# StevenChang5/Canny_Edge

Hardware: AMD Instinct MI355X
Metric: Mpixels/s device-resident Canny (4K gray, frames in HBM, whole pipeline); % HBM roofline on Sobel+NMS in `roofline`; the end-to-end (host->host, PCIe-inclusive) rate is `end_to_end` (higher is better)
Workload: dtype f32+s16; 1 GPU; 128x 3840x2160 gray frames per GPU per step, sigma=1.4, thresholds 50/150, inputs resident in HBM; frames_per_gpu=128, height=2160, width=3840

## Files before the change

### canny_edge_amd/csrc/canny_kernels.hip

```cpp
#include "canny_kernels.h"

#include <hip/hip_ext.h>

namespace canny {

__device__ __forceinline__ uint64_t shfl_up_u64(uint64_t v)
{
    unsigned lo = (unsigned)v, hi = (unsigned)(v >> 32);
    lo = __shfl_up(lo, 1);
    hi = __shfl_up(hi, 1);
    return ((uint64_t)hi << 32) | lo;
}
__device__ __forceinline__ uint64_t shfl_down_u64(uint64_t v)
{
    unsigned lo = (unsigned)v, hi = (unsigned)(v >> 32);
    lo = __shfl_down(lo, 1);
    hi = __shfl_down(hi, 1);
    return ((uint64_t)hi << 32) | lo;
}

__device__ __forceinline__ uint64_t readlane_u64(uint64_t v, int uniform_lane)
{
    const unsigned lo = (unsigned)__builtin_amdgcn_readlane((int)(unsigned)v, uniform_lane);
    const unsigned hi = (unsigned)__builtin_amdgcn_readlane((int)(unsigned)(v >> 32), uniform_lane);
    return ((uint64_t)hi << 32) | lo;
}

__device__ __forceinline__ uint64_t lane_u64(uint64_t v, int src_lane)
{
    unsigned lo = __shfl((unsigned)v, src_lane), hi = __shfl((unsigned)(v >> 32), src_lane);
    return ((uint64_t)hi << 32) | lo;
}

__device__ __forceinline__ int magnitude_general(int gx, int gy)
{
    long long n = (long long)gx * gx + (long long)gy * gy;
    return (int)(int16_t)(int)sqrt((double)n);
}
__device__ __forceinline__ int angle_bin_general(int gx, int gy)
{
    long long A = (long long)gx * gx, B = (long long)gy * gy, P = (long long)gx * gy;
    long long twoP = 2 * (P < 0 ? -P : P);
    if (twoP <= A - B) return 0;
    if (twoP < B - A) return 90;
    return P > 0 ? 45 : 135;
}
__device__ __forceinline__ int magnitude_d8(int gx, int gy)
{
    int n = __mul24(gx, gx) + __mul24(gy, gy);
    return (int)__builtin_amdgcn_sqrtf((float)n + 0.5f);
}
__device__ __forceinline__ int angle_bin_d8(int gx, int gy)
{
    int A = __mul24(gx, gx), B = __mul24(gy, gy), P = __mul24(gx, gy);
    int twoP = 2 * (P < 0 ? -P : P);
    int D = A - B;
    return (twoP <= D) ? 0 : ((twoP < -D) ? 90 : (P > 0 ? 45 : 135));
}

__device__ __forceinline__ void sobel_at(const int16_t *__restrict__ f, int H, int W, int r, int c, int &gx, int &gy)
{
    int cl = c > 0 ? c - 1 : 0, cr = c < W - 1 ? c + 1 : W - 1;
    int ru = r > 0 ? r - 1 : 0, rd = r < H - 1 ? r + 1 : H - 1;
    const int16_t *row = f + (size_t)r * W;
    const int16_t *up = f + (size_t)ru * W;
    const int16_t *dn = f + (size_t)rd * W;
    int v = 2 * row[cr] - 2 * row[cl];
    if (r < H - 1) v += dn[cr] - dn[cl];
    if (r > 0) v += up[cr] - up[cl];
    int u = 2 * dn[c] - 2 * up[c];
    if (c < W - 1) u += dn[c + 1] - up[c + 1];
    if (c > 0) u += dn[c - 1] - up[c - 1];
    gx = (int16_t)v;
    gy = (int16_t)u;
}

template <class At>
__device__ __forceinline__ void sobel_staged(const At &at, int H, int W, int r, int c, int ly, int lx, int &gx, int &gy)
{
    int lxl = c > 0 ? lx - 1 : lx, lxr = c < W - 1 ? lx + 1 : lx;
    int lyu = r > 0 ? ly - 1 : ly, lyd = r < H - 1 ? ly + 1 : ly;
    int v = 2 * at(ly, lxr) - 2 * at(ly, lxl);
    if (r < H - 1) v += at(ly + 1, lxr) - at(ly + 1, lxl);
    if (r > 0) v += at(ly - 1, lxr) - at(ly - 1, lxl);
    int u = 2 * at(lyd, lx) - 2 * at(lyu, lx);
    if (c < W - 1) u += at(lyd, lx + 1) - at(lyu, lx + 1);
    if (c > 0) u += at(lyd, lx - 1) - at(lyu, lx - 1);
    gx = (int16_t)v;
    gy = (int16_t)u;
}

__global__ __launch_bounds__(256) void gauss_rows_generic_kernel(const uint8_t *__restrict__ img,
                                                                 float *__restrict__ tmp, int W, size_t total,
                                                                 GaussTaps t)
{
    size_t stride = (size_t)gridDim.x * blockDim.x;
    for (size_t i = (size_t)blockIdx.x * blockDim.x + threadIdx.x; i < total; i += stride) {
        int c = (int)(i % (size_t)W);
        const uint8_t *row = img + (i - c);
        float acc = 0.0f, wsum = 0.0f;
        for (int k = -t.center; k <= t.center; k++) {
            int cc = c + k;
            if (cc >= 0 && cc < W) {
                float w = t.tap[t.center + k];
                acc = __fadd_rn(acc, __fmul_rn((float)row[cc], w));
                wsum = __fadd_rn(wsum, w);
            }
        }
        tmp[i] = __fdiv_rn(acc, wsum);
    }
}

__global__ __launch_bounds__(256) void gauss_cols_generic_kernel(const float *__restrict__ tmp,
                                                                 int16_t *__restrict__ out, int H, int W,
                                                                 size_t total, GaussTaps t)
{
    size_t stride = (size_t)gridDim.x * blockDim.x;
    for (size_t i = (size_t)blockIdx.x * blockDim.x + threadIdx.x; i < total; i += stride) {
        size_t rowidx = i / (size_t)W;
        int r = (int)(rowidx % (size_t)H);
        float acc = 0.0f, wsum = 0.0f;
        for (int k = -t.center; k <= t.center; k++) {
            int rr = r + k;
            if (rr >= 0 && rr < H) {
                float w = t.tap[t.center + k];
                acc = __fadd_rn(acc, __fmul_rn(tmp[i + (ptrdiff_t)k * W], w));
                wsum = __fadd_rn(wsum, w);
            }
        }
        out[i] = (int16_t)__fdiv_rn(acc, wsum);
    }
}

static inline unsigned grid_for(size_t total, int block, unsigned cap = 256u * 32u)
{
    size_t g = (total + block - 1) / block;
    if (g > cap) g = cap;
    if (g < 1) g = 1;
    return (unsigned)g;
}

hipError_t launch_gaussian_generic(const uint8_t *img, float *tmp, int16_t *out, int height, int width,
                                   int n_frames, const GaussTaps &taps, hipStream_t stream)
{
    size_t total = (size_t)n_frames * height * width;
    unsigned grid = grid_for(total, 256);
    hipLaunchKernelGGL(gauss_rows_generic_kernel, dim3(grid), dim3(256), 0, stream, img, tmp, width, total, taps);
    hipLaunchKernelGGL(gauss_cols_generic_kernel, dim3(grid), dim3(256), 0, stream, tmp, out, height, width, total,
                       taps);
    return hipGetLastError();
}


// ... 278 lines not shown
    int v[HG_PER_THREAD];
    auto fetch = [&](int t) {
        const int x0 = (t % tiles_x) * HG_TW, y0 = (t / tiles_x) * HG_TH;
#pragma unroll
        for (int k = 0; k < HG_PER_THREAD; k++) {
            const int i = (int)threadIdx.x + k * kHistWaves * 64;
            const int ly = i / (HG_TW + 2), lx = i - ly * (HG_TW + 2);
            const int r = y0 - 1 + ly, c = x0 - 1 + lx;
            v[k] = 0;
            if (t < tiles && i < HG_STAGE && r >= 0 && r < H && c >= 0 && c < W) {
                const size_t q = f * frame_px + (size_t)r * W + c;
                v[k] = U8 ? ((const uint8_t *)plane)[q] : ((const int16_t *)plane)[q];
            }
        }
    };
    fetch(blockIdx.x);
    for (int t = blockIdx.x; t < tiles; t += gridDim.x) {
        const int x0 = (t % tiles_x) * HG_TW, y0 = (t / tiles_x) * HG_TH;
        __syncthreads();
#pragma unroll
        for (int k = 0; k < HG_PER_THREAD; k++) {
            const int i = (int)threadIdx.x + k * kHistWaves * 64;
            if (i < HG_STAGE) (&tile[0][0])[i] = (int16_t)v[k];
        }
        __syncthreads();
        fetch(t + gridDim.x);
        for (int i = threadIdx.x; i < HG_TH * HG_TW; i += blockDim.x) {
            const int my = i / HG_TW, mx = i - my * HG_TW;
            const int r = y0 + my, c = x0 + mx;
            if (r >= H || c >= W) continue;
            int gx, gy;
            sobel_staged([&](int y, int x) -> int { return tile[y][x]; }, H, W, r, c, my + 1, mx + 1, gx, gy);
            wave_hist_add(h, min(magnitude_d8(gx, gy), kHistBins - 1));
        }
    }
    hist_flush(sh, hist + f * kHistBins);
}

static unsigned hist_blocks_per_frame(int n_frames, size_t units_per_frame)
{
    size_t b = ((size_t)kHistBlocks + n_frames - 1) / n_frames;
    if (b > units_per_frame) b = units_per_frame;
    return (unsigned)(b < 1 ? 1 : b);
}

hipError_t launch_hist_intensity(const void *plane, bool in_u8, uint32_t *hist, int height, int width, int n_frames,
                                 hipStream_t stream)
{
    const size_t frame_px = (size_t)height * width, total = frame_px * n_frames;
    const size_t lanes = (frame_px / 16 + 2 + kHistGroups - 1) / kHistGroups;
    const dim3 grid(hist_blocks_per_frame(n_frames, (lanes + kHistWaves * 64 - 1) / (kHistWaves * 64)), n_frames);
    if (in_u8)
        hipLaunchKernelGGL(hist_intensity_kernel<true>, grid, dim3(kHistWaves * 64), 0, stream, plane, hist, frame_px,
                           total);
    else
        hipLaunchKernelGGL(hist_intensity_kernel<false>, grid, dim3(kHistWaves * 64), 0, stream, plane, hist, frame_px,
                           total);
    return hipGetLastError();
}

hipError_t launch_hist_gradient(const void *plane, bool in_u8, uint32_t *hist, int height, int width, int n_frames,
                                hipStream_t stream)
{
    const size_t tiles = (size_t)((width + HG_TW - 1) / HG_TW) * ((height + HG_TH - 1) / HG_TH);
    const dim3 grid(hist_blocks_per_frame(n_frames, tiles), n_frames);
    if (in_u8)
        hipLaunchKernelGGL(hist_gradient_kernel<true>, grid, dim3(kHistWaves * 64), 0, stream, plane, hist, height,
                           width);
    else
        hipLaunchKernelGGL(hist_gradient_kernel<false>, grid, dim3(kHistWaves * 64), 0, stream, plane, hist, height,
                           width);
    return hipGetLastError();
}

__global__ __launch_bounds__(64) void thr_select_kernel(const uint32_t *__restrict__ hist, int rule, double low,
                                                        double high, int *__restrict__ pairs)
{
    __shared__ unsigned long long cs[kHistBins];
    const int f = blockIdx.x, lane = threadIdx.x;
    const uint32_t *hf = hist + (size_t)f * kHistBins;
    unsigned long long part[5], run = 0;
#pragma unroll
    for (int k = 0; k < 5; k++) {
        const int b = 5 * lane + k;
        run += b < kHistBins ? hf[b] : 0u;
        part[k] = run;
    }
    unsigned long long x = run;
    for (int d = 1; d < 64; d <<= 1) {
        const unsigned lo = __shfl_up((unsigned)x, d), hi = __shfl_up((unsigned)(x >> 32), d);
        if (lane >= d) x += ((unsigned long long)hi << 32) | lo;
    }
    const unsigned long long excl = x - run;
#pragma unroll
    for (int k = 0; k < 5; k++)
        if (5 * lane + k < kHistBins) cs[5 * lane + k] = excl + part[k];
    __syncthreads();
    if (lane == 0) {
        int lo, hi;
        auto_thresholds([&](int b) { return cs[b]; }, rule, low, high, lo, hi);
        pairs[2 * f] = lo;
        pairs[2 * f + 1] = hi;
    }
}

hipError_t launch_thr_select(const uint32_t *hist, int n_frames, int rule, double low, double high, int *pairs,
                             hipStream_t stream)
{
    hipLaunchKernelGGL(thr_select_kernel, dim3(n_frames), dim3(64), 0, stream, hist, rule, low, high, pairs);
    return hipGetLastError();
}

__device__ __forceinline__ size_t word_index(const HystGeom &g, int f, int y, int wx)
{
    return ((((size_t)f * g.tiles_y + (y >> 6)) * g.tiles_x + wx) << 6) + (y & 63);
}

template <bool THR>
__global__ __launch_bounds__(256) void hyst_classify_kernel(const int16_t *__restrict__ cand,
                                                            uint64_t *__restrict__ strong,
                                                            uint64_t *__restrict__ conn, HystGeom g, int lo, int hi,
                                                            unsigned *domain_flag, const int *__restrict__ pairs)
{
    const int lane = threadIdx.x & 63;
    const size_t rows_padded = (size_t)g.tiles_y * kTile;
    const size_t n_words = (size_t)g.n_frames * rows_padded * g.tiles_x;
    const size_t wave_stride = ((size_t)gridDim.x * blockDim.x) >> 6;
    for (size_t wv = ((size_t)blockIdx.x * blockDim.x + threadIdx.x) >> 6; wv < n_words; wv += wave_stride) {
        int wx = (int)(wv % (size_t)g.tiles_x);
        size_t t = wv / (size_t)g.tiles_x;
        int y = (int)(t % rows_padded);
        int f = (int)(t / rows_padded);
        if constexpr (THR) {
            lo = pairs[2 * f];
            hi = pairs[2 * f + 1];
            clamp_thresholds(lo, hi);
        }
        int x = wx * kTile + lane;
        bool inside = (y < g.height) && (x < g.width);
        int v = 0;
        if (inside) v = cand[((size_t)f * g.height + y) * g.width + x];
        bool c = inside && v >= lo;
        bool s = c && v >= hi;
        if (inside && lo <= 0 && v < lo) atomicOr(domain_flag, 1u);
        uint64_t mc = __ballot(c), ms = __ballot(s);
        if (lane == 0) {
            size_t idx = word_index(g, f, y, wx);
            conn[idx] = mc;
            strong[idx] = ms;
        }
    }
}

__device__ __forceinline__ uint64_t row_above_u64(uint64_t v)
{
    unsigned lo = (unsigned)__builtin_amdgcn_mov_dpp((int)(unsigned)v, 0x138 , 0xf, 0xf, true);
    unsigned hi = (unsigned)__builtin_amdgcn_mov_dpp((int)(unsigned)(v >> 32), 0x138, 0xf, 0xf, true);
    return ((uint64_t)hi << 32) | lo;
}
__device__ __forceinline__ uint64_t row_below_u64(uint64_t v)
{
    unsigned lo = (unsigned)__builtin_amdgcn_mov_dpp((int)(unsigned)v, 0x130 , 0xf, 0xf, true);
    unsigned hi = (unsigned)__builtin_amdgcn_mov_dpp((int)(unsigned)(v >> 32), 0x130, 0xf, 0xf, true);
    return ((uint64_t)hi << 32) | lo;
}

__device__ __forceinline__ uint64_t fill_runs(uint64_t p, uint64_t g)
{
    const uint64_t up = ((p + g) ^ p) & p;
    const uint64_t pr = __brevll(p), gr = __brevll(g);
    const uint64_t down = __brevll(((pr + gr) ^ pr) & pr);
    return g | up | down;
}

struct HystSched {
    unsigned *stamp, *queue0, *queue1, *count;
    unsigned *fq0, *fq1, *fcount;
};
constexpr int kSweep0Tiles = 2;
__device__ __forceinline__ HystSched make_sched(unsigned *words, int tiles)
{
    HystSched s;
    s.stamp = words;
    s.queue0 = words + tiles;
    s.queue1 = words + 2 * (size_t)tiles;
    s.count = words + 3 * (size_t)tiles;
    s.fq0 = words + 3 * (size_t)tiles + 4;
    s.fq1 = words + 4 * (size_t)tiles + 4;
    s.fcount = words + 5 * (size_t)tiles + 4;
    return s;
}

struct TileIn {
    uint64_t s0, su, sd;
    unsigned lb, rb;
    unsigned ul, ur, dl, dr;
};

constexpr uint64_t kAllHalo = ~0ull;
__device__ __forceinline__ TileIn load_tile(int t, int lane, const uint64_t *__restrict__ strong, const HystGeom &g,
                                            uint64_t c = kAllHalo)
{
    const int tpf = g.tiles_x * g.tiles_y;
    const int tt = t % tpf;
    const int ty = tt / g.tiles_x, tx = tt - ty * g.tiles_x;
    const uint64_t c_top = readlane_u64(c, 0), c_bot = readlane_u64(c, 63);
    const bool needL = __any((c & 1ull) != 0), needR = __any((c >> 63) != 0);
    const bool hasU = ty > 0 && c_top != 0, hasD = ty < g.tiles_y - 1 && c_bot != 0;
    const bool hasL = tx > 0 && needL, hasR = tx < g.tiles_x - 1 && needR;
    const size_t base = (size_t)t * kTile;
    const size_t rowstep = (size_t)g.tiles_x * kTile;
    TileIn in;
    in.s0 = strong[base + lane];
    in.su = hasU ? strong[base - rowstep + 63] : 0;
    in.sd = hasD ? strong[base + rowstep] : 0;
    in.lb = hasL ? (unsigned)(strong[base - kTile + lane] >> 63) : 0u;
    in.rb = hasR ? (unsigned)(strong[base + kTile + lane] & 1u) : 0u;
    in.ul = (hasU && hasL && (c_top & 1ull)) ? (unsigned)(strong[base - rowstep - kTile + 63] >> 63) : 0u;
    in.ur = (hasU && hasR && (c_top >> 63)) ? (unsigned)(strong[base - rowstep + kTile + 63] & 1u) : 0u;
    in.dl = (hasD && hasL && (c_bot & 1ull)) ? (unsigned)(strong[base + rowstep - kTile] >> 63) : 0u;
    in.dr = (hasD && hasR && (c_bot >> 63)) ? (unsigned)(strong[base + rowstep + kTile] & 1u) : 0u;
    return in;
}

__device__ __forceinline__ void push_neighbours(bool want, int lane, unsigned *stamp, unsigned slot, unsigned entry,
                                                unsigned nxt, unsigned *q, unsigned *cnt)
{
    const bool won = want && atomicExch(&stamp[slot], nxt) != nxt;
    const uint64_t winners = __ballot(won);
    if (winners == 0) return;
    unsigned first = 0;
    if (lane == 0) first = atomicAdd(cnt, (unsigned)__popcll(winners));
    first = (unsigned)__builtin_amdgcn_readlane((int)first, 0);
    if (won) q[first + (unsigned)__popcll(winners & ((1ull << lane) - 1ull))] = entry;
}

template <class Push>
__device__ __forceinline__ void process_tile_with(int t, int lane, uint64_t *__restrict__ strong, int iter,
                                                  const HystGeom &g, int16_t *__restrict__ edges, int edge_value,
                                                  uint64_t c, const TileIn &in, Push push_tiles)
{
    const int tpf = g.tiles_x * g.tiles_y;
    const int tt = t % tpf;
    const int ty = tt / g.tiles_x, tx = tt - ty * g.tiles_x;
    const bool hasU = ty > 0, hasD = ty < g.tiles_y - 1, hasL = tx > 0, hasR = tx < g.tiles_x - 1;
    const size_t base = (size_t)t * kTile;
    const uint64_t s0 = in.s0, su = in.su, sd = in.sd;
    const unsigned lb = in.lb, rb = in.rb, ul = in.ul, ur = in.ur, dl = in.dl, dr = in.dr;
    unsigned lb_up = __shfl_up(lb, 1), lb_dn = __shfl_down(lb, 1);
    unsigned rb_up = __shfl_up(rb, 1), rb_dn = __shfl_down(rb, 1);
    if (lane == 0) { lb_up = ul; rb_up = ur; }
    if (lane == 63) { lb_dn = dl; rb_dn = dr; }
    const uint64_t in_left = (uint64_t)(lb | lb_up | lb_dn);
    const uint64_t in_right = (uint64_t)(rb | rb_up | rb_dn) << 63;
    const bool quirk = (ty == 0 && tx == 0 && lane == 0);

    uint64_t s = s0;
    for (;;) {
        uint64_t up = row_above_u64(s), dn = row_below_u64(s);
        if (lane == 0) up = su;
        if (lane == 63) dn = sd;
        uint64_t d = up | s | dn;
        uint64_t d_from_left = quirk ? (up | s | (dn & ~1ull)) : d;
        uint64_t nb = d | (d_from_left << 1) | (d >> 1) | in_left | in_right;
        uint64_t gsel = s | (c & nb);
        if (!__any(gsel != s)) break;
        s = fill_runs(c, gsel);
    }

    const uint64_t chg = s ^ s0;
    const uint64_t rows_changed = __ballot(chg != 0);
    if (rows_changed != 0) {
        strong[base + lane] = s;
        if (edges) {
            const int f = t / tpf;
            const int cols = min(kTile, g.width - tx * kTile), rows = min(kTile, g.height - ty * kTile);
            int16_t *const tile0 = edges + ((size_t)f * g.height + (size_t)ty * kTile) * g.width + tx * kTile;
            if (__popcll(rows_changed) <= 16) {
                for (uint64_t m = rows_changed; m != 0; m &= m - 1) {
                    const int r = __builtin_ctzll(m);
                    const uint64_t word = readlane_u64(chg, r);
                    if (((word >> lane) & 1ull) != 0 && lane < cols && r < rows)
                        tile0[(size_t)r * g.width + lane] = (int16_t)edge_value;
                }
            } else if (lane < rows) {
                int16_t *const rowp = tile0 + (size_t)lane * g.width;
                for (uint64_t m = chg; m != 0; m &= m - 1) {
                    const int b = __builtin_ctzll(m);
                    if (b < cols) rowp[b] = (int16_t)edge_value;
                }
            }
        }
        const uint64_t top64 = readlane_u64(chg, 0);
        const uint64_t bot = readlane_u64(chg, 63);
        const bool anyL = __any((chg & 1ull) != 0), anyR = __any((chg >> 63) != 0);
        const int dy = (lane == 0 || lane == 4 || lane == 5) ? -1 : ((lane == 1 || lane == 6 || lane == 7) ? 1 : 0);
        const int dx = (lane == 2 || lane == 4 || lane == 6) ? -1 : ((lane == 3 || lane == 5 || lane == 7) ? 1 : 0);
        const uint64_t facing = dy < 0 ? top64 : bot;
        const bool hit = dy == 0 ? (dx < 0 ? anyL : anyR)
                                 : (dx == 0 ? facing != 0 : (dx < 0 ? (facing & 1ull) != 0 : (facing >> 63) != 0));
        const bool there = (dy >= 0 || hasU) && (dy <= 0 || hasD) && (dx >= 0 || hasL) && (dx <= 0 || hasR);
        const bool want = lane < 8 && hit && there;
        push_tiles(want, t + dy * g.tiles_x + dx);
    }
}

__device__ __forceinline__ void note_push(unsigned *last_change, unsigned nxt)
{
    if (__hip_atomic_load(last_change, __ATOMIC_RELAXED, __HIP_MEMORY_SCOPE_AGENT) < nxt) atomicMax(last_change, nxt);
}

__device__ __forceinline__ void process_tile(int t, int lane, uint64_t *__restrict__ strong, const HystSched &sch,
                                             unsigned *__restrict__ last_change, int iter, const HystGeom &g,
                                             int16_t *__restrict__ edges, int edge_value, uint64_t c,
                                             const TileIn &in, bool to_frame = false)
{
    const unsigned nxt = (unsigned)iter + 1u;
    unsigned *q = (nxt & 1u) ? sch.queue1 : sch.queue0;
    unsigned *cnt = sch.count + nxt % 3u;
    if (to_frame) {
        const int tpf = g.tiles_x * g.tiles_y;
        const int f = t / tpf;
        q = ((nxt & 1u) ? sch.fq1 : sch.fq0) + (size_t)f * tpf;
        cnt = sch.fcount + 4 * (size_t)f + nxt % 3u;
    }
    process_tile_with(t, lane, strong, iter, g, edges, edge_value, c, in, [&](bool want, int nb) {
        push_neighbours(want, lane, sch.stamp, (unsigned)nb, (unsigned)nb, nxt, q, cnt);
        if (__any(want) && lane == 0) note_push(last_change, nxt);
    });
}

__device__ __forceinline__ void propagate_tile(int t, int lane, uint64_t *__restrict__ strong,
                                               const uint64_t *__restrict__ conn, const HystSched &sch,
                                               unsigned *__restrict__ last_change, int iter, const HystGeom &g,
                                               int16_t *__restrict__ edges, int edge_value, uint64_t c,
                                               bool to_frame = false)
{
    if (!__any(c != 0)) return;
    const TileIn in = load_tile(t, lane, strong, g, c);
    process_tile(t, lane, strong, sch, last_change, iter, g, edges, edge_value, c, in, to_frame);
}

__global__ __launch_bounds__(256) void hyst_propagate_kernel(uint64_t *__restrict__ strong,
                                                             const uint64_t *__restrict__ conn,
                                                             unsigned *__restrict__ sched_words,
                                                             unsigned *__restrict__ last_change, int iter, HystGeom g,
                                                             int16_t *__restrict__ edges, int edge_value,
                                                             int frame_groups)
{
    const int lane = threadIdx.x & 63;
    const int wave = __builtin_amdgcn_readfirstlane(blockIdx.x * 4 + (threadIdx.x >> 6));
    const int n_waves = gridDim.x * 4;
    const int tiles = g.tiles();
    const HystSched sch = make_sched(sched_words, tiles);
    if (wave == 0 && lane == 0) sch.count[(iter + 2) % 3] = 0;
    if (iter == 0) {
        for (int t0 = wave * kSweep0Tiles; t0 < tiles; t0 += n_waves * kSweep0Tiles) {
            uint64_t c[kSweep0Tiles];
#pragma unroll
            for (int k = 0; k < kSweep0Tiles; k++)
                c[k] = (t0 + k < tiles) ? conn[(size_t)(t0 + k) * kTile + lane] : 0ull;
#pragma unroll
            for (int k = 0; k < kSweep0Tiles; k++)
                propagate_tile(t0 + k, lane, strong, conn, sch, last_change, iter, g, edges, edge_value, c[k],
                               frame_groups > 0);
        }
        return;
    }
    if (frame_groups > 0) {
        const int tpf = g.tiles_x * g.tiles_y;
        const int f = (int)blockIdx.x / frame_groups, part = (int)blockIdx.x - f * frame_groups;
        unsigned *const fcount = sch.fcount + 4 * (size_t)f;
        if (part == 0 && threadIdx.x == 0) fcount[(iter + 2) % 3] = 0;
        const unsigned n = min(__hip_atomic_load(fcount + iter % 3, __ATOMIC_RELAXED, __HIP_MEMORY_SCOPE_AGENT),
                               (unsigned)tpf);
        const unsigned *q = ((iter & 1) ? sch.fq1 : sch.fq0) + (size_t)f * tpf;
        const unsigned w = (unsigned)__builtin_amdgcn_readfirstlane(part * 4 + (int)(threadIdx.x >> 6));
        for (unsigned i = w; i < n; i += (unsigned)frame_groups * 4u) {
            const int t = (int)q[i];
            propagate_tile(t, lane, strong, conn, sch, last_change, iter, g, edges, edge_value,
                           conn[(size_t)t * kTile + lane], true);
        }
        return;
    }
    const unsigned n = __hip_atomic_load(sch.count + iter % 3, __ATOMIC_RELAXED, __HIP_MEMORY_SCOPE_AGENT);
    const unsigned *q = (iter & 1) ? sch.queue1 : sch.queue0;
    for (unsigned i = (unsigned)wave; i < n; i += (unsigned)n_waves) {
        const int t = (int)q[i];
        propagate_tile(t, lane, strong, conn, sch, last_change, iter, g, edges, edge_value,
                       conn[(size_t)t * kTile + lane]);
    }
}

constexpr int kTailTiles = 4096;
__global__ __launch_bounds__(1024) void hyst_tail_kernel(uint64_t *__restrict__ strong, const uint64_t *__restrict__ conn,
                                                         unsigned *__restrict__ sched_words,
                                                         unsigned *__restrict__ last_change, int first_iter, HystGeom g,
                                                         int16_t *__restrict__ edges, int edge_value)
{
    __shared__ unsigned s_queue[2][kTailTiles];
    __shared__ unsigned s_stamp[kTailTiles];
    __shared__ unsigned s_count[2];
    __shared__ unsigned s_last;
    const int lane = threadIdx.x & 63;
    const int wave = __builtin_amdgcn_readfirstlane(threadIdx.x >> 6), n_waves = blockDim.x >> 6;
    const int f = blockIdx.x;
    const int tpf = g.tiles_x * g.tiles_y;
    const int t_base = f * tpf;
    const HystSched sch = make_sched(sched_words, g.tiles());
    int cur = first_iter & 1;
    {
        const unsigned n0 = __hip_atomic_load(sch.fcount + 4 * (size_t)f + first_iter % 3, __ATOMIC_RELAXED,
                                              __HIP_MEMORY_SCOPE_AGENT);
        const unsigned *q0 = (cur ? sch.fq1 : sch.fq0) + (size_t)t_base;
        for (unsigned i = threadIdx.x; i < n0; i += blockDim.x)
            s_queue[cur][i] = __hip_atomic_load(q0 + i, __ATOMIC_RELAXED, __HIP_MEMORY_SCOPE_AGENT) - (unsigned)t_base;
        for (int i = threadIdx.x; i < tpf; i += blockDim.x) s_stamp[i] = 0;
        if (threadIdx.x == 0) {
            s_count[cur] = n0;
            s_count[cur ^ 1] = 0;
            s_last = 0;
        }
    }
    unsigned pushed = 0;
    for (int iter = first_iter;; iter++, cur ^= 1) {
        __syncthreads();
        const unsigned n = s_count[cur];
        __syncthreads();
        if (n == 0) break;
        if (threadIdx.x == 0) s_count[cur] = 0;
        unsigned *const q_next = s_queue[cur ^ 1];
        unsigned *const n_next = &s_count[cur ^ 1];
        const unsigned nxt = (unsigned)iter + 1u;
        for (unsigned i = (unsigned)wave; i < n; i += (unsigned)n_waves) {
            const int t = t_base + (int)s_queue[cur][i];
            const uint64_t c = conn[(size_t)t * kTile + lane];
            const TileIn in = load_tile(t, lane, strong, g);
            if (!__any(c != 0)) continue;
            process_tile_with(t, lane, strong, iter, g, edges, edge_value, c, in, [&](bool want, int nb) {
                const unsigned loc = (unsigned)(nb - t_base);
                push_neighbours(want, lane, s_stamp, loc, loc, nxt, q_next, n_next);
                if (__any(want)) pushed = nxt;
            });
        }
    }
    if (lane == 0 && pushed != 0) atomicMax(&s_last, pushed);
    __syncthreads();
    if (threadIdx.x == 0 && s_last != 0) atomicMax(last_change, s_last);
}

__global__ __launch_bounds__(256) void hyst_finalize_kernel(int16_t *__restrict__ cand,
                                                            const uint64_t *__restrict__ strong, HystGeom g,
                                                            int edge_value)
{
    const size_t plane = (size_t)g.height * g.width;
    const size_t total = plane * g.n_frames;
    const size_t stride = (size_t)gridDim.x * blockDim.x;
    for (size_t i = (size_t)blockIdx.x * blockDim.x + threadIdx.x; i < total; i += stride) {
        size_t f = i / plane, p = i - f * plane;
        int y = (int)(p / (size_t)g.width), x = (int)(p - (size_t)y * g.width);
        uint64_t w = strong[word_index(g, (int)f, y, x >> 6)];
        cand[i] = ((w >> (x & 63)) & 1ull) ? (int16_t)edge_value : (int16_t)0;
    }
}

__global__ __launch_bounds__(256) void fep_classify_kernel(const int16_t *__restrict__ cand,
                                                           const uint8_t *__restrict__ visited,
                                                           uint64_t *__restrict__ strong, uint64_t *__restrict__ conn,
                                                           HystGeom g, int start, int lo)
{
    const int lane = threadIdx.x & 63;
    const size_t rows_padded = (size_t)g.tiles_y * kTile;
    const size_t n_words = rows_padded * g.tiles_x;
    const size_t wave_stride = ((size_t)gridDim.x * blockDim.x) >> 6;
    for (size_t wv = ((size_t)blockIdx.x * blockDim.x + threadIdx.x) >> 6; wv < n_words; wv += wave_stride) {
        int wx = (int)(wv % (size_t)g.tiles_x);
        int y = (int)(wv / (size_t)g.tiles_x);
        int x = wx * kTile + lane;
        bool inside = (y < g.height) && (x < g.width);
        bool c = false, s = false;
        if (inside) {
            size_t i = (size_t)y * g.width + x;
            s = ((long long)i == (long long)start);
            c = s || (cand[i] >= lo && !visited[i]);
        }
        uint64_t mc = __ballot(c), ms = __ballot(s);
        if (lane == 0) {
            size_t idx = word_index(g, 0, y, wx);
            conn[idx] = mc;
            strong[idx] = ms;
        }
    }
}

__device__ __forceinline__ bool bit_at(const uint64_t *planeS, const HystGeom &g, int y, int x)
{
    if (y < 0 || y >= g.height || x < 0 || x >= g.width) return false;
    return (planeS[word_index(g, 0, y, x >> 6)] >> (x & 63)) & 1ull;
}

__global__ __launch_bounds__(256) void fep_finalize_kernel(int16_t *__restrict__ cand, uint8_t *__restrict__ visited,
                                                           const uint64_t *__restrict__ strong, HystGeom g, int start,
                                                           int lo)
{
    const size_t total = (size_t)g.height * g.width;
    const size_t stride = (size_t)gridDim.x * blockDim.x;
    for (size_t i = (size_t)blockIdx.x * blockDim.x + threadIdx.x; i < total; i += stride) {
        int y = (int)(i / (size_t)g.width), x = (int)(i - (size_t)y * g.width);
        if (!bit_at(strong, g, y, x)) continue;
        cand[i] = 255;
        if ((long long)i != (long long)start) {
            visited[i] = 1;
        } else if (255 >= lo) {
            bool pushed = false;
            for (int dy = -1; dy <= 1; dy++)
                for (int dx = -1; dx <= 1; dx++) {
                    if (!dy && !dx) continue;
                    int py = y + dy, px = x + dx;
                    if (!bit_at(strong, g, py, px)) continue;
                    if (py == 1 && px == 0 && y == 0 && x == 1) continue;
                    pushed = true;
                }
            if (pushed) visited[i] = 1;
        }
    }
}

__device__ __forceinline__ uint32_t pk_sub_sat_i16(uint32_t a, uint32_t b)
{
    typedef short s16x2_t __attribute__((ext_vector_type(2)));
    return __builtin_bit_cast(uint32_t, __builtin_elementwise_sub_sat(__builtin_bit_cast(s16x2_t, a),
                                                                      __builtin_bit_cast(s16x2_t, b)));
}

constexpr int kPatchItems = 4;
__device__ __forceinline__ bool patch_coords(const HystGeom &g, int k, size_t &i, int &f, int &y, int &x0)
{
    const int tx = (int)blockIdx.x * 2 + (k >> 1), ty = (int)blockIdx.y;
    const int within = (k & 1) * 256 + (int)threadIdx.x;
    f = (int)blockIdx.z;
    i = ((((size_t)f * g.tiles_y + ty) * g.tiles_x + tx) << 9) + within;
    y = ty * kTile + (within >> 3);
    x0 = tx * kTile + (within & 7) * 8;
    return tx < g.tiles_x && y < g.height && x0 < g.width;
}
__device__ __forceinline__ bool patch_tile_exists(const HystGeom &g, int k)
{
    return (int)blockIdx.x * 2 + (k >> 1) < g.tiles_x;
}

template <bool THR>
__global__ __launch_bounds__(256) void hyst_classify8_kernel(const int16_t *__restrict__ cand,
                                                             uint8_t *__restrict__ strong, uint8_t *__restrict__ conn,
                                                             HystGeom g, int lo, int hi, unsigned *domain_flag,
                                                             const int *__restrict__ pairs)
{
    if constexpr (THR) {
        lo = pairs[2 * blockIdx.z];
        hi = pairs[2 * blockIdx.z + 1];
        clamp_thresholds(lo, hi);
    }
    const bool fast = lo >= -32768 && lo <= 32767 && hi >= -32768 && hi <= 32767;
    const uint32_t lo2 = ((uint32_t)lo & 0xffffu) * 0x10001u, hi2 = ((uint32_t)hi & 0xffffu) * 0x10001u;
    uint4 px4[kPatchItems];
    size_t idx[kPatchItems];
    bool inside[kPatchItems];
#pragma unroll
    for (int k = 0; k < kPatchItems; k++) {
        int f, y, x0;
        inside[k] = patch_coords(g, k, idx[k], f, y, x0);
        px4[k] = make_uint4(0u, 0u, 0u, 0u);
        if (inside[k]) __builtin_memcpy(&px4[k], cand + ((size_t)f * g.height + y) * g.width + x0, 16);
    }
#pragma unroll
    for (int k = 0; k < kPatchItems; k++) {
        if (!patch_tile_exists(g, k)) continue;
        const size_t i = idx[k];
        unsigned cbits = 0, sbits = 0;
        if (inside[k]) {
            const uint4 v = px4[k];
            const uint32_t w[4] = {v.x, v.y, v.z, v.w};
            if (fast) {
                const uint32_t r[4] = {__builtin_amdgcn_perm(w[2], w[0], 0x05040100u),
                                       __builtin_amdgcn_perm(w[2], w[0], 0x07060302u),
                                       __builtin_amdgcn_perm(w[3], w[1], 0x05040100u),
                                       __builtin_amdgcn_perm(w[3], w[1], 0x07060302u)};
                uint32_t dc[4], ds[4];
#pragma unroll
                for (int k = 0; k < 4; k++) {
                    const uint32_t a = pk_sub_sat_i16(r[k], lo2);
                    const uint32_t b = pk_sub_sat_i16(r[k], hi2);
                    dc[k] = a & 0x80008000u;
// ... 43 lines not shown
    }
}

hipError_t launch_hyst_classify(const int16_t *cand, uint64_t *strong, uint64_t *conn, const HystGeom &g, int min_val,
                                int max_val, unsigned *domain_flag, hipStream_t stream, const int *pairs)
{
    size_t n_words = (size_t)g.n_frames * g.tiles_y * kTile * g.tiles_x;
    const dim3 grid8((g.tiles_x + 1) / 2, g.tiles_y, g.n_frames), grid(grid_for(n_words * 64, 256));
    if (g.width % 8 == 0 && pairs)
        hipLaunchKernelGGL(hyst_classify8_kernel<true>, grid8, dim3(256), 0, stream, cand, (uint8_t *)strong,
                           (uint8_t *)conn, g, min_val, max_val, domain_flag, pairs);
    else if (g.width % 8 == 0)
        hipLaunchKernelGGL(hyst_classify8_kernel<false>, grid8, dim3(256), 0, stream, cand, (uint8_t *)strong,
                           (uint8_t *)conn, g, min_val, max_val, domain_flag, pairs);
    else if (pairs)
        hipLaunchKernelGGL(hyst_classify_kernel<true>, grid, dim3(256), 0, stream, cand, strong, conn, g, min_val,
                           max_val, domain_flag, pairs);
    else
        hipLaunchKernelGGL(hyst_classify_kernel<false>, grid, dim3(256), 0, stream, cand, strong, conn, g, min_val,
                           max_val, domain_flag, pairs);
    return hipGetLastError();
}
__global__ __launch_bounds__(256) void hyst_prepare_kernel(uint64_t *__restrict__ strong, uint64_t *__restrict__ conn,
                                                           HystGeom g, int pad_waves, unsigned *__restrict__ sched,
                                                           unsigned n_sched, unsigned *__restrict__ flags,
                                                           int n_flags)
{
    const int lane = (int)(threadIdx.x & 63);
    const int wave = (int)blockIdx.x * 4 + (int)(threadIdx.x >> 6);
    if (wave < pad_waves) {
        const int per_frame = g.tiles_x + g.tiles_y;
        const int f = wave / per_frame, k = wave - f * per_frame;
        const int tx = k < g.tiles_x ? k : g.tiles_x - 1;
        const int ty = k < g.tiles_x ? g.tiles_y - 1 : k - g.tiles_x;
        const size_t w = ((((size_t)f * g.tiles_y + ty) * g.tiles_x + tx) << 6) + lane;
        const int y = ty * kTile + lane;
        const int valid_px = min(kTile, g.width - tx * kTile);
        if (y >= g.height) {
            strong[w] = 0;
            conn[w] = 0;
        } else if (valid_px < kTile) {
            uint8_t *sb = (uint8_t *)(strong + w), *cb = (uint8_t *)(conn + w);
            for (int b = valid_px / 8; b < 8; b++) sb[b] = cb[b] = 0;
        }
        return;
    }
    const size_t i0 = ((size_t)(wave - pad_waves) * 64 + lane) * 4;
    for (int j = 0; j < 4; j++)
        if (i0 + j < n_sched) sched[i0 + j] = 0u;
    if (wave == pad_waves && lane < n_flags) flags[lane] = 0u;
}

hipError_t launch_hyst_prepare(uint64_t *strong, uint64_t *conn, const HystGeom &g, bool zero_pad, unsigned *sched,
                               unsigned *flags, hipStream_t stream, int n_lanes)
{
    if (n_lanes < 1 || n_lanes > 16) return hipErrorInvalidValue;
    const bool pad = zero_pad && (g.height % kTile != 0 || g.width % kTile != 0);
    const long long pad_waves = pad ? (long long)(g.tiles_x + g.tiles_y) * g.n_frames : 0;
    const size_t n_sched = 5 * (size_t)g.tiles() + 4 * (size_t)n_lanes + 4 * (size_t)g.n_frames;
    const long long waves = pad_waves + (long long)((n_sched + 255) / 256);
    if (pad_waves > 0x3fffffffLL || n_sched > 0xffffffffull) return hipErrorInvalidValue;
    hipLaunchKernelGGL(hyst_prepare_kernel, dim3((unsigned)((waves + 3) / 4)), dim3(256), 0, stream, strong, conn, g,
                       (int)pad_waves, sched, (unsigned)n_sched, flags, 2 * n_lanes);
    return hipGetLastError();
}

__global__ __launch_bounds__(256) void edges_to_u8_kernel(const int16_t *__restrict__ in, uint8_t *__restrict__ out,
                                                          size_t n)
{
    const size_t groups = n / 16;
    const size_t stride = (size_t)gridDim.x * blockDim.x;
    const bool aligned = (((uintptr_t)in | (uintptr_t)out) & 15u) == 0;
    for (size_t g = (size_t)blockIdx.x * blockDim.x + threadIdx.x; g < groups; g += stride) {
        if (aligned) {
            const uint4 a = *reinterpret_cast<const uint4 *>(in + g * 16);
            const uint4 b = *reinterpret_cast<const uint4 *>(in + g * 16 + 8);
            uint4 r;
            r.x = __builtin_amdgcn_perm(a.y, a.x, 0x06040200u);
            r.y = __builtin_amdgcn_perm(a.w, a.z, 0x06040200u);
            r.z = __builtin_amdgcn_perm(b.y, b.x, 0x06040200u);
            r.w = __builtin_amdgcn_perm(b.w, b.z, 0x06040200u);
            *reinterpret_cast<uint4 *>(out + g * 16) = r;
        } else {
            for (int k = 0; k < 16; k++) out[g * 16 + k] = (uint8_t)in[g * 16 + k];
        }
    }
    if (blockIdx.x == 0 && threadIdx.x < n % 16) out[groups * 16 + threadIdx.x] = (uint8_t)in[groups * 16 + threadIdx.x];
}

hipError_t launch_edges_to_u8(const int16_t *edges, uint8_t *out, size_t n, hipStream_t stream)
{
    if (n == 0) return hipSuccess;
    hipLaunchKernelGGL(edges_to_u8_kernel, dim3(grid_for(n / 16 + 1, 256)), dim3(256), 0, stream, edges, out, n);
    return hipGetLastError();
}

__global__ __launch_bounds__(256) void edges_to_bits_kernel(const int16_t *__restrict__ in, uint8_t *__restrict__ out,
                                                            int width, int row_bytes, size_t n_bytes, int vec_ok)
{
    const size_t stride = (size_t)gridDim.x * blockDim.x;
    for (size_t b = (size_t)blockIdx.x * blockDim.x + threadIdx.x; b < n_bytes; b += stride) {
        const size_t row = b / (size_t)row_bytes;
        const int xb = (int)(b - row * (size_t)row_bytes);
        const int16_t *px = in + row * (size_t)width + (size_t)xb * 8;
        unsigned byte = 0;
        if (vec_ok) {
            const uint4 v = *reinterpret_cast<const uint4 *>(px);
            const unsigned d[4] = {v.x, v.y, v.z, v.w};
#pragma unroll
            for (int k = 0; k < 4; k++)
                byte |= (((d[k] & 0xffffu) != 0 ? 2u : 0u) | ((d[k] >> 16) != 0 ? 1u : 0u)) << (6 - 2 * k);
        } else {
            const int left = width - xb * 8;
#pragma unroll
            for (int k = 0; k < 8; k++)
                if (k < left && px[k] != 0) byte |= 0x80u >> k;
        }
        out[b] = (uint8_t)byte;
    }
}

hipError_t launch_edges_to_bits(const int16_t *edges, uint8_t *bits, int height, int width, int n_frames,
                                hipStream_t stream)
{
    const int row_bytes = (width + 7) / 8;
    const size_t n_bytes = (size_t)n_frames * (size_t)height * (size_t)row_bytes;
    if (n_bytes == 0) return hipSuccess;
    const int vec_ok = (width % 8 == 0) && (((uintptr_t)edges & 15u) == 0);
    hipLaunchKernelGGL(edges_to_bits_kernel, dim3(grid_for(n_bytes, 256)), dim3(256), 0, stream, edges, bits, width,
                       row_bytes, n_bytes, vec_ok);
    return hipGetLastError();
}

__global__ void hyst_publish_kernel(const unsigned *__restrict__ flags, unsigned *host, unsigned seq)
{
    __hip_atomic_store(&host[0], flags[0], __ATOMIC_RELAXED, __HIP_MEMORY_SCOPE_SYSTEM);
    __hip_atomic_store(&host[1], flags[1], __ATOMIC_RELAXED, __HIP_MEMORY_SCOPE_SYSTEM);
    __hip_atomic_store(&host[2], seq, __ATOMIC_RELEASE, __HIP_MEMORY_SCOPE_SYSTEM);
}

hipError_t launch_hyst_publish(const unsigned *flags, unsigned *host_flags_dev, unsigned seq, hipStream_t stream)
{
    hipLaunchKernelGGL(hyst_publish_kernel, dim3(1), dim3(1), 0, stream, flags, host_flags_dev, seq);
    return hipGetLastError();
}

hipError_t launch_hyst_tail(uint64_t *strong, const uint64_t *conn, unsigned *sched, unsigned *last_change,
                            int first_iter, const HystGeom &g, hipStream_t stream, int16_t *edges, int edge_value)
{
    if (g.n_frames < 1 || first_iter < 1 || g.tiles_x * g.tiles_y > kTailTiles) return hipErrorInvalidValue;
    const int tpf = g.tiles_x * g.tiles_y;
    const unsigned threads = tpf >= 256 ? 1024u : (tpf >= 64 ? 512u : 256u);
    hipLaunchKernelGGL(hyst_tail_kernel, dim3((unsigned)g.n_frames), dim3(threads), 0, stream, strong, conn, sched,
                       last_change, first_iter, g, edges, edge_value);
    return hipGetLastError();
}

hipError_t launch_hyst_propagate(uint64_t *strong, const uint64_t *conn, unsigned *stamp, unsigned *last_change,
                                 int iter, const HystGeom &g, hipStream_t stream, int16_t *edges, int edge_value,
                                 bool frame_queues)
{
    if (frame_queues && (g.n_frames < 1 || g.tiles_x * g.tiles_y > kTailTiles)) return hipErrorInvalidValue;
    unsigned blocks = (unsigned)((g.tiles() + 4 * kSweep0Tiles - 1) / (4 * kSweep0Tiles));
    int frame_groups = frame_queues ? 1 : 0;
    if (iter > 0) {
        const unsigned want = (unsigned)((g.tiles() + 15) / 16);
        blocks = want < 8u ? 8u : (want > 1024u ? 1024u : want);
        if (frame_queues) {
            frame_groups = (int)(blocks / (unsigned)g.n_frames);
            if (frame_groups < 1) frame_groups = 1;
            blocks = (unsigned)frame_groups * (unsigned)g.n_frames;
        }
    }
    hipLaunchKernelGGL(hyst_propagate_kernel, dim3(blocks), dim3(256), 0, stream, strong, conn, stamp, last_change,
                       iter, g, edges, edge_value, frame_groups);
    return hipGetLastError();
}
__global__ __launch_bounds__(256) void hyst_finalize_rows_kernel(int16_t *__restrict__ cand,
                                                                 const uint8_t *__restrict__ strong, HystGeom g,
                                                                 int edge_value, int groups_per_row)
{
    const uint32_t ev = (uint32_t)(uint16_t)edge_value;
    const int chunk = (int)blockIdx.x * 4 + (int)(threadIdx.x >> 6);
    const int gx = chunk * 64 + (int)(threadIdx.x & 63);
    if (gx >= groups_per_row) return;
    const int f = (int)blockIdx.z;
    const int x0 = gx * 8;
    const size_t tile_col = ((size_t)f * g.tiles_y) * g.tiles_x + (gx >> 3);
    unsigned b[4];
#pragma unroll
    for (int k = 0; k < 4; k++) {
        const int y = (int)blockIdx.y * 4 + k;
        b[k] = 0;
        if (y < g.height)
            b[k] = strong[((tile_col + (size_t)(y >> 6) * g.tiles_x) << 9) + (size_t)(y & 63) * 8 + (gx & 7)];
    }
#pragma unroll
    for (int k = 0; k < 4; k++) {
        const int y = (int)blockIdx.y * 4 + k;
        if (y >= g.height) break;
        const uint32_t t = b[k] | (b[k] << 15);
        uint4 v;
        v.x = __umul24(t & 0x00010001u, ev);
        v.y = __umul24((t >> 2) & 0x00010001u, ev);
        v.z = __umul24((t >> 4) & 0x00010001u, ev);
        v.w = __umul24((t >> 6) & 0x00010001u, ev);
        __builtin_memcpy(cand + ((size_t)f * g.height + y) * g.width + x0, &v, 16);
    }
}

static int finalize_mode = 0;
void hyst_set_finalize_mode(int m) { finalize_mode = m; }

hipError_t launch_hyst_finalize(int16_t *cand, const uint64_t *strong, const HystGeom &g, int edge_value,
                                hipStream_t stream)
{
    size_t total = (size_t)g.n_frames * g.height * g.width;
    if (g.width % 8 == 0 && finalize_mode != 1) {
        const int groups = g.width / 8;
        hipLaunchKernelGGL(hyst_finalize_rows_kernel, dim3((groups + 255) / 256, (g.height + 3) / 4, g.n_frames),
                           dim3(256), 0, stream, cand, (const uint8_t *)strong, g, edge_value, groups);
    } else if (g.width % 8 == 0)
        hipLaunchKernelGGL(hyst_finalize8_kernel, dim3((g.tiles_x + 1) / 2, g.tiles_y, g.n_frames), dim3(256), 0, stream, cand,
                           (const uint8_t *)strong, g, edge_value);
    else
        hipLaunchKernelGGL(hyst_finalize_kernel, dim3(grid_for(total, 256)), dim3(256), 0, stream, cand, strong, g,
                           edge_value);
    return hipGetLastError();
}
hipError_t launch_fep_classify(const int16_t *cand, const uint8_t *visited, uint64_t *strong, uint64_t *conn,
                               const HystGeom &g, int start, int min_val, hipStream_t stream)
{
    size_t n_words = (size_t)g.tiles_y * kTile * g.tiles_x;
    hipLaunchKernelGGL(fep_classify_kernel, dim3(grid_for(n_words * 64, 256)), dim3(256), 0, stream, cand, visited,
                       strong, conn, g, start, min_val);
    return hipGetLastError();
}
hipError_t launch_fep_finalize(int16_t *cand, uint8_t *visited, const uint64_t *strong, const HystGeom &g, int start,
                               int min_val, hipStream_t stream)
{
    size_t total = (size_t)g.height * g.width;
    hipLaunchKernelGGL(fep_finalize_kernel, dim3(grid_for(total, 256)), dim3(256), 0, stream, cand, visited, strong, g,
                       start, min_val);
    return hipGetLastError();
}

__global__ __launch_bounds__(256) void selftest_mag_angle_kernel(int lim, int16_t *__restrict__ mags,
                                                                 uint8_t *__restrict__ bins)
{
    const int side = 2 * lim + 1;
    const size_t total = (size_t)side * side;
    const size_t stride = (size_t)gridDim.x * blockDim.x;
    for (size_t i = (size_t)blockIdx.x * blockDim.x + threadIdx.x; i < total; i += stride) {
        int gy = (int)(i / side) - lim, gx = (int)(i % side) - lim;
        mags[i] = (int16_t)magnitude_d8(gx, gy);
        bins[i] = (uint8_t)angle_bin_d8(gx, gy);
    }
}
hipError_t launch_selftest_mag_angle(int lim, int16_t *mags, uint8_t *bins, hipStream_t stream)
{
    size_t total = (size_t)(2 * lim + 1) * (2 * lim + 1);
    hipLaunchKernelGGL(selftest_mag_angle_kernel, dim3(grid_for(total, 256)), dim3(256), 0, stream, lim, mags, bins);
    return hipGetLastError();
}


__global__ __launch_bounds__(256) void probe_copy_kernel(const uint4 *__restrict__ in, uint4 *__restrict__ out, size_t n16)
{
    const size_t i = (size_t)blockIdx.x * 256 + threadIdx.x;
    if (i < n16) out[i] = in[i];
}
hipError_t launch_probe_copy(const void *src, void *dst, size_t nbytes, hipStream_t stream, const LaunchEvents &ev)
{
    const size_t n16 = nbytes / 16;
    if (n16 == 0) return hipSuccess;
    const size_t blocks = (n16 + 255) / 256;
    if (blocks > 0x7fffffffu) return hipErrorInvalidValue;
    if (ev.start && ev.stop)
        hipExtLaunchKernelGGL(probe_copy_kernel, dim3((unsigned)blocks), dim3(256), 0, stream, ev.start, ev.stop, 0,
                              (const uint4 *)src, (uint4 *)dst, n16);
    else
        hipLaunchKernelGGL(probe_copy_kernel, dim3((unsigned)blocks), dim3(256), 0, stream, (const uint4 *)src,
                           (uint4 *)dst, n16);
    return hipGetLastError();
}

}
```

Before: 595,300 Mpixels/s.

## Precompute tile coordinates with magic division and trim hysteresis tile-load overhead

Replaces the integer divide and modulo that recover frame, tile row and tile column in the hysteresis kernels with host-precomputed multiply-shift division. Consecutive tiles in the first sweep are advanced incrementally. Halo bits are now read as 32-bit halves instead of full 64-bit words, and lane shuffles use DPP row moves. Queue pointer selection moves into the push lambda, and the propagate kernel is pinned to 8 waves per EU. All of this cuts scalar and vector ALU work and register pressure in the latency-bound propagation loop. It risks a correctness bug if the magic divisor is inexact for large tile indices, and the occupancy pin may force register spills.

```diff
diff --git a/canny_edge_amd/csrc/canny_kernels.hip b/canny_edge_amd/csrc/canny_kernels.hip
--- a/canny_edge_amd/csrc/canny_kernels.hip
+++ b/canny_edge_amd/csrc/canny_kernels.hip
@@ -1,4 +1,5 @@
 #include "canny_kernels.h"
+#include "canny_tile_div.h"
 
 #include <hip/hip_ext.h>
 
@@ -583,17 +584,21 @@
     }
 }
 
+__device__ __forceinline__ unsigned row_above_u32(unsigned v)
+{
+    return (unsigned)__builtin_amdgcn_mov_dpp((int)v, 0x138 , 0xf, 0xf, true);
+}
+__device__ __forceinline__ unsigned row_below_u32(unsigned v)
+{
+    return (unsigned)__builtin_amdgcn_mov_dpp((int)v, 0x130 , 0xf, 0xf, true);
+}
 __device__ __forceinline__ uint64_t row_above_u64(uint64_t v)
 {
-    unsigned lo = (unsigned)__builtin_amdgcn_mov_dpp((int)(unsigned)v, 0x138 , 0xf, 0xf, true);
-    unsigned hi = (unsigned)__builtin_amdgcn_mov_dpp((int)(unsigned)(v >> 32), 0x138, 0xf, 0xf, true);
-    return ((uint64_t)hi << 32) | lo;
+    return ((uint64_t)row_above_u32((unsigned)(v >> 32)) << 32) | row_above_u32((unsigned)v);
 }
 __device__ __forceinline__ uint64_t row_below_u64(uint64_t v)
 {
-    unsigned lo = (unsigned)__builtin_amdgcn_mov_dpp((int)(unsigned)v, 0x130 , 0xf, 0xf, true);
-    unsigned hi = (unsigned)__builtin_amdgcn_mov_dpp((int)(unsigned)(v >> 32), 0x130, 0xf, 0xf, true);
-    return ((uint64_t)hi << 32) | lo;
+    return ((uint64_t)row_below_u32((unsigned)(v >> 32)) << 32) | row_below_u32((unsigned)v);
 }
 
 __device__ __forceinline__ uint64_t fill_runs(uint64_t p, uint64_t g)
@@ -622,6 +627,46 @@
     return s;
 }
 
+struct TilePos {
+    int t, f, ty, tx;
+};
+struct HystDiv {
+    TileDiv by_frame, by_row;
+};
+inline HystDiv make_hyst_div(const HystGeom &g)
+{
+    HystDiv dv;
+    dv.by_frame = make_tile_div(g.tiles_x * g.tiles_y);
+    dv.by_row = make_tile_div(g.tiles_x);
+    return dv;
+}
+__device__ __forceinline__ TilePos tile_pos(int t, int f, int tt, const HystGeom &g, const HystDiv &dv)
+{
+    TilePos p;
+    p.t = t;
+    p.f = f;
+    p.ty = (int)tile_div((unsigned)tt, dv.by_row);
+    p.tx = tt - p.ty * g.tiles_x;
+    return p;
+}
+__device__ __forceinline__ TilePos tile_pos(int t, const HystGeom &g, const HystDiv &dv)
+{
+    const int f = (int)tile_div((unsigned)t, dv.by_frame);
+    return tile_pos(t, f, t - f * (g.tiles_x * g.tiles_y), g, dv);
+}
+__device__ __forceinline__ TilePos next_tile(TilePos p, const HystGeom &g)
+{
+    p.t++;
+    if (++p.tx == g.tiles_x) {
+        p.tx = 0;
+        if (++p.ty == g.tiles_y) {
+            p.ty = 0;
+            p.f++;
+        }
+    }
+    return p;
+}
+
 struct TileIn {
     uint64_t s0, su, sd;
     unsigned lb, rb;
@@ -629,28 +674,37 @@
 };
 
 constexpr uint64_t kAllHalo = ~0ull;
-__device__ __forceinline__ TileIn load_tile(int t, int lane, const uint64_t *__restrict__ strong, const HystGeom &g,
-                                            uint64_t c = kAllHalo)
-{
-    const int tpf = g.tiles_x * g.tiles_y;
-    const int tt = t % tpf;
-    const int ty = tt / g.tiles_x, tx = tt - ty * g.tiles_x;
+__device__ __forceinline__ TileIn load_tile(const TilePos &p, int lane, const uint64_t *__restrict__ strong,
+                                            const HystGeom &g, uint64_t c = kAllHalo)
+{
+    const int ty = p.ty, tx = p.tx;
     const uint64_t c_top = readlane_u64(c, 0), c_bot = readlane_u64(c, 63);
     const bool needL = __any((c & 1ull) != 0), needR = __any((c >> 63) != 0);
     const bool hasU = ty > 0 && c_top != 0, hasD = ty < g.tiles_y - 1 && c_bot != 0;
     const bool hasL = tx > 0 && needL, hasR = tx < g.tiles_x - 1 && needR;
-    const size_t base = (size_t)t * kTile;
     const size_t rowstep = (size_t)g.tiles_x * kTile;
+    const uint64_t *const own = strong + (size_t)p.t * kTile, *const up = own - rowstep, *const dn = own + rowstep;
     TileIn in;
-    in.s0 = strong[base + lane];
-    in.su = hasU ? strong[base - rowstep + 63] : 0;
-    in.sd = hasD ? strong[base + rowstep] : 0;
-    in.lb = hasL ? (unsigned)(strong[base - kTile + lane] >> 63) : 0u;
-    in.rb = hasR ? (unsigned)(strong[base + kTile + lane] & 1u) : 0u;
-    in.ul = (hasU && hasL && (c_top & 1ull)) ? (unsigned)(strong[base - rowstep - kTile + 63] >> 63) : 0u;
-    in.ur = (hasU && hasR && (c_top >> 63)) ? (unsigned)(strong[base - rowstep + kTile + 63] & 1u) : 0u;
-    in.dl = (hasD && hasL && (c_bot & 1ull)) ? (unsigned)(strong[base + rowstep - kTile] >> 63) : 0u;
-    in.dr = (hasD && hasR && (c_bot >> 63)) ? (unsigned)(strong[base + rowstep + kTile] & 1u) : 0u;
+    in.s0 = own[lane];
+    in.su = hasU ? up[63] : 0;
+    in.sd = hasD ? dn[0] : 0;
+    typedef unsigned __attribute__((may_alias)) half_t;
+    auto hi = [](const uint64_t *word) { return ((const half_t *)word)[1]; };
+    auto lo = [](const uint64_t *word) { return ((const half_t *)word)[0]; };
+    unsigned wl = 0, wr = 0, wul = 0, wur = 0, wdl = 0, wdr = 0;
+    if (hasL) wl = hi(own - kTile + lane);
+    if (hasR) wr = lo(own + kTile + lane);
+    if (hasU && hasL && (c_top & 1ull)) wul = hi(up - kTile + 63);
+    if (hasU && hasR && (c_top >> 63)) wur = lo(up + kTile + 63);
+    if (hasD && hasL && (c_bot & 1ull)) wdl = hi(dn - kTile);
+    if (hasD && hasR && (c_bot >> 63)) wdr = lo(dn + kTile);
+    asm volatile("" : "+v"(wl), "+v"(wr), "+v"(wul), "+v"(wur), "+v"(wdl), "+v"(wdr));
+    in.lb = wl >> 31;
+    in.rb = wr & 1u;
+    in.ul = wul >> 31;
+    in.ur = wur & 1u;
+    in.dl = wdl >> 31;
+    in.dr = wdr & 1u;
     return in;
 }
 
@@ -667,19 +721,17 @@
 }
 
 template <class Push>
-__device__ __forceinline__ void process_tile_with(int t, int lane, uint64_t *__restrict__ strong, int iter,
+__device__ __forceinline__ void process_tile_with(const TilePos &p, int lane, uint64_t *__restrict__ strong, int iter,
                                                   const HystGeom &g, int16_t *__restrict__ edges, int edge_value,
                                                   uint64_t c, const TileIn &in, Push push_tiles)
 {
-    const int tpf = g.tiles_x * g.tiles_y;
-    const int tt = t % tpf;
-    const int ty = tt / g.tiles_x, tx = tt - ty * g.tiles_x;
+    const int t = p.t, ty = p.ty, tx = p.tx;
     const bool hasU = ty > 0, hasD = ty < g.tiles_y - 1, hasL = tx > 0, hasR = tx < g.tiles_x - 1;
     const size_t base = (size_t)t * kTile;
     const uint64_t s0 = in.s0, su = in.su, sd = in.sd;
     const unsigned lb = in.lb, rb = in.rb, ul = in.ul, ur = in.ur, dl = in.dl, dr = in.dr;
-    unsigned lb_up = __shfl_up(lb, 1), lb_dn = __shfl_down(lb, 1);
-    unsigned rb_up = __shfl_up(rb, 1), rb_dn = __shfl_down(rb, 1);
+    unsigned lb_up = row_above_u32(lb), lb_dn = row_below_u32(lb);
+    unsigned rb_up = row_above_u32(rb), rb_dn = row_below_u32(rb);
     if (lane == 0) { lb_up = ul; rb_up = ur; }
     if (lane == 63) { lb_dn = dl; rb_dn = dr; }
     const uint64_t in_left = (uint64_t)(lb | lb_up | lb_dn);
@@ -704,7 +756,7 @@
     if (rows_changed != 0) {
         strong[base + lane] = s;
         if (edges) {
-            const int f = t / tpf;
+            const int f = p.f;
             const int cols = min(kTile, g.width - tx * kTile), rows = min(kTile, g.height - ty * kTile);
             int16_t *const tile0 = edges + ((size_t)f * g.height + (size_t)ty * kTile) * g.width + tx * kTile;
             if (__popcll(rows_changed) <= 16) {
@@ -741,42 +793,40 @@
     if (__hip_atomic_load(last_change, __ATOMIC_RELAXED, __HIP_MEMORY_SCOPE_AGENT) < nxt) atomicMax(last_change, nxt);
 }
 
-__device__ __forceinline__ void process_tile(int t, int lane, uint64_t *__restrict__ strong, const HystSched &sch,
+__device__ __forceinline__ void process_tile(const TilePos &p, int lane, uint64_t *__restrict__ strong, const HystSched &sch,
                                              unsigned *__restrict__ last_change, int iter, const HystGeom &g,
                                              int16_t *__restrict__ edges, int edge_value, uint64_t c,
                                              const TileIn &in, bool to_frame = false)
 {
     const unsigned nxt = (unsigned)iter + 1u;
-    unsigned *q = (nxt & 1u) ? sch.queue1 : sch.queue0;
-    unsigned *cnt = sch.count + nxt % 3u;
-    if (to_frame) {
-        const int tpf = g.tiles_x * g.tiles_y;
-        const int f = t / tpf;
-        q = ((nxt & 1u) ? sch.fq1 : sch.fq0) + (size_t)f * tpf;
-        cnt = sch.fcount + 4 * (size_t)f + nxt % 3u;
-    }
-    process_tile_with(t, lane, strong, iter, g, edges, edge_value, c, in, [&](bool want, int nb) {
+    process_tile_with(p, lane, strong, iter, g, edges, edge_value, c, in, [&](bool want, int nb) {
+        unsigned *q = (nxt & 1u) ? sch.queue1 : sch.queue0;
+        unsigned *cnt = sch.count + nxt % 3u;
+        if (to_frame) {
+            q = ((nxt & 1u) ? sch.fq1 : sch.fq0) + (size_t)p.f * (g.tiles_x * g.tiles_y);
+            cnt = sch.fcount + 4 * (size_t)p.f + nxt % 3u;
+        }
         push_neighbours(want, lane, sch.stamp, (unsigned)nb, (unsigned)nb, nxt, q, cnt);
         if (__any(want) && lane == 0) note_push(last_change, nxt);
     });
 }
 
-__device__ __forceinline__ void propagate_tile(int t, int lane, uint64_t *__restrict__ strong,
+__device__ __forceinline__ void propagate_tile(const TilePos &p, int lane, uint64_t *__restrict__ strong,
                                                const uint64_t *__restrict__ conn, const HystSched &sch,
                                                unsigned *__restrict__ last_change, int iter, const HystGeom &g,
                                                int16_t *__restrict__ edges, int edge_value, uint64_t c,
                                                bool to_frame = false)
 {
     if (!__any(c != 0)) return;
-    const TileIn in = load_tile(t, lane, strong, g, c);
-    process_tile(t, lane, strong, sch, last_change, iter, g, edges, edge_value, c, in, to_frame);
-}
-
-__global__ __launch_bounds__(256) void hyst_propagate_kernel(uint64_t *__restrict__ strong,
+    const TileIn in = load_tile(p, lane, strong, g, c);
+    process_tile(p, lane, strong, sch, last_change, iter, g, edges, edge_value, c, in, to_frame);
+}
+
+__global__ __launch_bounds__(256) __attribute__((amdgpu_waves_per_eu(8, 8))) void hyst_propagate_kernel(uint64_t *__restrict__ strong,
                                                              const uint64_t *__restrict__ conn,
                                                              unsigned *__restrict__ sched_words,
                                                              unsigned *__restrict__ last_change, int iter, HystGeom g,
-                                                             int16_t *__restrict__ edges, int edge_value,
+                                                             HystDiv dv, int16_t *__restrict__ edges, int edge_value,
                                                              int frame_groups)
 {
     const int lane = threadIdx.x & 63;
@@ -791,10 +841,13 @@
 #pragma unroll
             for (int k = 0; k < kSweep0Tiles; k++)
                 c[k] = (t0 + k < tiles) ? conn[(size_t)(t0 + k) * kTile + lane] : 0ull;
-#pragma unroll
-            for (int k = 0; k < kSweep0Tiles; k++)
-                propagate_tile(t0 + k, lane, strong, conn, sch, last_change, iter, g, edges, edge_value, c[k],
+            TilePos p = tile_pos(t0, g, dv);
+#pragma unroll
+            for (int k = 0; k < kSweep0Tiles; k++) {
+                if (k > 0) p = next_tile(p, g);
+                propagate_tile(p, lane, strong, conn, sch, last_change, iter, g, edges, edge_value, c[k],
                                frame_groups > 0);
+            }
         }
         return;
     }
@@ -809,8 +862,8 @@
         const unsigned w = (unsigned)__builtin_amdgcn_readfirstlane(part * 4 + (int)(threadIdx.x >> 6));
         for (unsigned i = w; i < n; i += (unsigned)frame_groups * 4u) {
             const int t = (int)q[i];
-            propagate_tile(t, lane, strong, conn, sch, last_change, iter, g, edges, edge_value,
-                           conn[(size_t)t * kTile + lane], true);
+            propagate_tile(tile_pos(t, f, t - f * tpf, g, dv), lane, strong, conn, sch, last_change, iter, g, edges,
+                           edge_value, conn[(size_t)t * kTile + lane], true);
         }
         return;
     }
@@ -818,7 +871,7 @@
     const unsigned *q = (iter & 1) ? sch.queue1 : sch.queue0;
     for (unsigned i = (unsigned)wave; i < n; i += (unsigned)n_waves) {
         const int t = (int)q[i];
-        propagate_tile(t, lane, strong, conn, sch, last_change, iter, g, edges, edge_value,
+        propagate_tile(tile_pos(t, g, dv), lane, strong, conn, sch, last_change, iter, g, edges, edge_value,
                        conn[(size_t)t * kTile + lane]);
     }
 }
@@ -827,7 +880,7 @@
 __global__ __launch_bounds__(1024) void hyst_tail_kernel(uint64_t *__restrict__ strong, const uint64_t *__restrict__ conn,
                                                          unsigned *__restrict__ sched_words,
                                                          unsigned *__restrict__ last_change, int first_iter, HystGeom g,
-                                                         int16_t *__restrict__ edges, int edge_value)
+                                                         HystDiv dv, int16_t *__restrict__ edges, int edge_value)
 {
     __shared__ unsigned s_queue[2][kTailTiles];
     __shared__ unsigned s_stamp[kTailTiles];
@@ -864,11 +917,13 @@
         unsigned *const n_next = &s_count[cur ^ 1];
         const unsigned nxt = (unsigned)iter + 1u;
         for (unsigned i = (unsigned)wave; i < n; i += (unsigned)n_waves) {
-            const int t = t_base + (int)s_queue[cur][i];
+            const int tt = (int)s_queue[cur][i];
+            const int t = t_base + tt;
+            const TilePos p = tile_pos(t, f, tt, g, dv);
             const uint64_t c = conn[(size_t)t * kTile + lane];
-            const TileIn in = load_tile(t, lane, strong, g);
+            const TileIn in = load_tile(p, lane, strong, g);
             if (!__any(c != 0)) continue;
-            process_tile_with(t, lane, strong, iter, g, edges, edge_value, c, in, [&](bool want, int nb) {
+            process_tile_with(p, lane, strong, iter, g, edges, edge_value, c, in, [&](bool want, int nb) {
                 const unsigned loc = (unsigned)(nb - t_base);
                 push_neighbours(want, lane, s_stamp, loc, loc, nxt, q_next, n_next);
                 if (__any(want)) pushed = nxt;
@@ -1218,7 +1273,7 @@
     const int tpf = g.tiles_x * g.tiles_y;
     const unsigned threads = tpf >= 256 ? 1024u : (tpf >= 64 ? 512u : 256u);
     hipLaunchKernelGGL(hyst_tail_kernel, dim3((unsigned)g.n_frames), dim3(threads), 0, stream, strong, conn, sched,
-                       last_change, first_iter, g, edges, edge_value);
+                       last_change, first_iter, g, make_hyst_div(g), edges, edge_value);
     return hipGetLastError();
 }
 
@@ -1239,7 +1294,7 @@
         }
     }
     hipLaunchKernelGGL(hyst_propagate_kernel, dim3(blocks), dim3(256), 0, stream, strong, conn, stamp, last_change,
-                       iter, g, edges, edge_value, frame_groups);
+                       iter, g, make_hyst_div(g), edges, edge_value, frame_groups);
     return hipGetLastError();
 }
 __global__ __launch_bounds__(256) void hyst_finalize_rows_kernel(int16_t *__restrict__ cand,
diff --git a/canny_edge_amd/csrc/canny_tile_div.h b/canny_edge_amd/csrc/canny_tile_div.h
--- /dev/null
+++ b/canny_edge_amd/csrc/canny_tile_div.h
@@ -0,0 +1,31 @@
+#pragma once
+
+#include <stdint.h>
+
+#if defined(__HIPCC__)
+#define CANNY_TILE_DIV_FN __host__ __device__ inline
+#else
+#define CANNY_TILE_DIV_FN inline
+#endif
+
+namespace canny {
+
+struct TileDiv {
+    uint32_t mul, shift;
+};
+
+inline TileDiv make_tile_div(int d)
+{
+    TileDiv v;
+    v.shift = 0;
+    while ((UINT32_C(1) << v.shift) < (uint32_t)d) v.shift++;
+    v.mul = (uint32_t)(((UINT64_C(1) << (31 + v.shift)) + (uint32_t)d - 1) / (uint32_t)d);
+    return v;
+}
+
+CANNY_TILE_DIV_FN uint32_t tile_div(uint32_t n, TileDiv v)
+{
+    return (uint32_t)(((uint64_t)(n << 1) * v.mul) >> 32) >> v.shift;
+}
+
+}
```

After: 603,600 Mpixels/s (median of 6 runs). 1.01x the previous value.
